# tijiang13/InstantAvatar

Hardware: NVIDIA H100
Metric: rays/sec at 512x512 render (higher is better)
Workload: dtype f32 geometry + f16 hash-grid/MLP (fp32 accumulate)

## Files before the change

### instantavatar_b200/csrc/ia_host.h

```cpp
#pragma once
#include <cuda_runtime.h>
#include <stdio.h>

#include "../../include/ia_b200.h"

char* ia_err_buf();

inline int ia_set_err(int code, const char* fmt, const char* detail = "") {
    snprintf(ia_err_buf(), 512, fmt, detail);
    return code;
}
#define set_err ia_set_err
#define IA_CHECK_CUDA(expr)                                                                        \
    do {                                                                                           \
        cudaError_t _e = (expr);                                                                   \
        if (_e != cudaSuccess) return ia_set_err(IA_ECUDA, #expr ": %s", cudaGetErrorString(_e)); \
    } while (0)
#define IA_REQUIRE(cond)                                                        \
    do {                                                                        \
        if (!(cond)) return ia_set_err(IA_EINVAL, "invalid argument: %s", #cond); \
    } while (0)

constexpr int kMaxDevices = 64;
inline int current_device() {
    int dev = 0;
    if (cudaGetDevice(&dev) != cudaSuccess) return -1;
    return dev;
}

inline int sm_count() {
    static int g_sm_count[kMaxDevices] = {};
    const int dev = current_device();
    if (dev < 0) return 0;
    int& c = g_sm_count[dev % kMaxDevices];
    if (!c) cudaDeviceGetAttribute(&c, cudaDevAttrMultiProcessorCount, dev);
    return c;
}

struct PerDeviceFlag {
    bool done[kMaxDevices] = {};
    bool get() const { const int d = current_device(); return d >= 0 && done[d % kMaxDevices]; }
    void set() { const int d = current_device(); if (d >= 0) done[d % kMaxDevices] = true; }
};

template <auto Kernel>
inline int allow_dynamic_smem(int bytes) {
    static PerDeviceFlag done;
    if (!done.get()) {
        IA_CHECK_CUDA(cudaFuncSetAttribute(Kernel, cudaFuncAttributeMaxDynamicSharedMemorySize, bytes));
        done.set();
    }
    return IA_OK;
}
```

### instantavatar_b200/csrc/ia_kernels.cu

```cuda
#include <math.h>
#include <stdio.h>
#include <string.h>

#include <type_traits>

#include "ia_warp_eval.cuh"

using namespace ia;

static int g_render_rays = 4;

constexpr int kRenderWarps = 12;

#include "ia_host.h"
#include "ia_scene.cuh"

static thread_local char g_err[512] = "";
char* ia_err_buf() { return g_err; }

struct RenderArgs {
    SceneDev sd;
    const float* rays_o; const float* rays_d; const float* near; const float* far; const float* bg;
    int n_rays, image_width;
    float* rgb; float* depth; float* alpha; float* counter;
    int* tile_counter;
    IaStats* stats;
    const int* tile_order;
    const int* n_active;
    const int* gidx; float* const* peer_rgba; int n_peers;
};

__device__ __forceinline__ void peer_store_rgba(const RenderArgs& a, int ray, float r, float g, float b, float al) {
    if (!a.peer_rgba) return;
    const long px = a.gidx ? a.gidx[ray] : ray;
    const float4 v = make_float4(r, g, b, al);
    for (int p = 0; p < a.n_peers; p++) reinterpret_cast<float4*>(a.peer_rgba[p])[px] = v;
}

struct RenderWarpExtra {
    float qx[64], qy[64], qz[64], qt[64];
    int qowner[64];
    float bt[32];
    int bo[32];
};

template <bool kNV = false>
struct RenderSmem {
    __align__(128) uint32_t occ[64 * 64 * 64 / 32];
    __align__(16) __half W[kMlpHalfs];
    FrameConst fc;
    __align__(8) uint64_t mbar;
    std::conditional_t<kNV, WarpScratchNV, WarpScratch<false>> ws[kRenderWarps];
    RenderWarpExtra wx[kRenderWarps];
};

__device__ __forceinline__ void occupied_interval(const FrameConst& fc, const int* __restrict__ cbox, int G, float ox,
                                                  float oy, float oz, float dx, float dy, float dz, float& t0, float& t1) {
    t0 = -INFINITY; t1 = INFINITY;
    const float o[3] = {ox, oy, oz}, d[3] = {dx, dy, dz};
#pragma unroll
    for (int a = 0; a < 3; a++) {
        const float cell = 1.0f / fc.occ_s[a];
        float lo = -INFINITY, hi = INFINITY;
        if (cbox[a] > 0) lo = fc.occ_min[a] + ((float)cbox[a] - 0.5f) * cell;
        if (cbox[3 + a] < G - 1) hi = fc.occ_min[a] + ((float)cbox[3 + a] + 1.5f) * cell;
        if (fabsf(d[a]) < 1e-12f) {
            if (o[a] < lo || o[a] > hi) { t0 = INFINITY; t1 = -INFINITY; }
        } else {
            const float inv = 1.0f / d[a];
            float ta = (lo - o[a]) * inv, tb = (hi - o[a]) * inv;
            if (ta > tb) { const float tmp = ta; ta = tb; tb = tmp; }
            if (ta == ta) t0 = fmaxf(t0, ta);
            if (tb == tb) t1 = fminf(t1, tb);
        }
    }
}

struct FrameRay {
    float ox = 0, oy = 0, oz = 0, dx = 0, dy = 0, dz = 1, t = 0, far = 0, dt = 0;
    int kbeg = 0, kend = -1;
};

__device__ __forceinline__ bool load_ray(const RenderArgs& a, const FrameConst& fc, const int* __restrict__ cbox, int G, int ray,
                                         FrameRay& r) {
    r.ox = a.rays_o[ray * 3]; r.oy = a.rays_o[ray * 3 + 1]; r.oz = a.rays_o[ray * 3 + 2];
    r.dx = a.rays_d[ray * 3]; r.dy = a.rays_d[ray * 3 + 1]; r.dz = a.rays_d[ray * 3 + 2];
    r.t = a.near[ray]; r.far = a.far[ray];
    r.dt = (r.far - r.t) / (float)IA_MAX_SAMPLES;
    float t0, t1;
    occupied_interval(fc, cbox, G, r.ox, r.oy, r.oz, r.dx, r.dy, r.dz, t0, t1);
    if (!(cbox[6] != 0 && t0 <= t1 && r.dt > 0.f)) return false;
    const float k0f = floorf((fmaxf(t0, r.t) - r.t) / r.dt) - 2.f, k1f = ceilf((fminf(t1, r.far) - r.t) / r.dt) + 2.f;
    r.kbeg = (int)fminf(fmaxf(k0f, 0.f), 1024.f);
    r.kend = (int)fminf(fmaxf(k1f, -1.f), 1024.f);
    return true;
}

__device__ __forceinline__ void store_ray(const RenderArgs& a, int ray, float Cr, float Cg, float Cb, float T, float Dp, float n) {
    float b0 = 1.f, b1 = 1.f, b2 = 1.f;
    if (a.bg) { b0 = a.bg[ray * 3]; b1 = a.bg[ray * 3 + 1]; b2 = a.bg[ray * 3 + 2]; }
    const float r = Cr + T * b0, g = Cg + T * b1, b = Cb + T * b2, al = 1.0f - T;
    a.rgb[ray * 3 + 0] = r; a.rgb[ray * 3 + 1] = g; a.rgb[ray * 3 + 2] = b;
    a.depth[ray] = Dp; a.alpha[ray] = al; a.counter[ray] = n;
    peer_store_rgba(a, ray, r, g, b, al);
}

__host__ __device__ constexpr int tile_width(int rays) { return rays >= 2 ? 2 : 1; }

template <int kRays>
__device__ __forceinline__ int tile_ray(int tile, int rl, bool tiled, int image_width) {
    constexpr int kTileW = tile_width(kRays);
    if (tiled) {
        const int tiles_x = image_width / kTileW;
        const int ty = tile / tiles_x, tx = tile % tiles_x;
        return (ty * (kRays / kTileW) + rl / kTileW) * image_width + tx * kTileW + (rl % kTileW);
    }
    return tile * kRays + rl;
}

template <int kRays, bool kNV = false>
__global__ void __launch_bounds__(256) render_plan_kernel(const __grid_constant__ RenderArgs a, int* __restrict__ cost) {
    __shared__ FrameConst fc;
    load_frame_const<kNV>(fc, a.sd);
    __syncthreads();
    constexpr int kTileW = tile_width(kRays);
    constexpr int kTileH = kRays / kTileW;
    const int G = a.sd.s.G;
    const uint32_t* occ = a.sd.s.occ_bits;
    const int* cbox = reinterpret_cast<const int*>(occ + G * G * G / 32);
    const bool tiled = a.image_width > 0 && (a.image_width % kTileW) == 0 && (a.n_rays % (a.image_width * kTileH)) == 0;
    const int n_tiles = (a.n_rays + kRays - 1) / kRays;
    const int gid = blockIdx.x * blockDim.x + threadIdx.x;
    const int tile = gid / kRays, rl = gid % kRays;
    int cnt = 0, ray = -1;
    if (tile < n_tiles) {
        ray = tile_ray<kRays>(tile, rl, tiled, a.image_width);
        if (ray < a.n_rays) {
            FrameRay r;
            if (load_ray(a, fc, cbox, G, ray, r)) {
                float t = r.t;
                for (int i = 0; i < r.kbeg; i++) t += r.dt;
                for (int k = r.kbeg; k <= r.kend && t < r.far; k++) {
                    const float x = __fmaf_rn(t, r.dx, r.ox), y = __fmaf_rn(t, r.dy, r.oy), z = __fmaf_rn(t, r.dz, r.oz);
                    cnt += occupied<true>(occ, fc.occ_min, fc.occ_s, G, x, y, z);
                    t += r.dt;
                }
            }
        } else {
            ray = -1;
        }
    }
    int tot = cnt;
#pragma unroll
    for (int o = 1; o < kRays; o <<= 1) tot += __shfl_xor_sync(kFull, tot, o);
    if (tile < n_tiles) {
        if (rl == 0) cost[tile] = tot;
        if (tot == 0 && ray >= 0) store_ray(a, ray, 0.f, 0.f, 0.f, 1.f, 0.f, 0.f);
    }
}

__global__ void __launch_bounds__(1024) order_tiles_kernel(const int* __restrict__ cost, int n_tiles, int* __restrict__ order,
                                                           int* __restrict__ n_active) {
    __shared__ int hist[256];
    __shared__ int offs[256];
    constexpr int kPer = 16;
    for (int i = threadIdx.x; i < 256; i += blockDim.x) hist[i] = 0;
    __syncthreads();
    auto bucket = [](int c) { return 255 - min(255, c >> 2); };
    for (int base = 0; base < n_tiles; base += 1024 * kPer) {
        int c[kPer];
#pragma unroll
        for (int j = 0; j < kPer; j++) { const int i = base + j * 1024 + threadIdx.x; c[j] = i < n_tiles ? cost[i] : 0; }
#pragma unroll
        for (int j = 0; j < kPer; j++) if (c[j] > 0) atomicAdd(&hist[bucket(c[j])], 1);
    }
    __syncthreads();
    if (threadIdx.x < 32) {
        int loc[8], sum = 0;
#pragma unroll
        for (int j = 0; j < 8; j++) { loc[j] = hist[threadIdx.x * 8 + j]; sum += loc[j]; }
        int incl = sum;
        for (int o = 1; o < 32; o <<= 1) { const int y = __shfl_up_sync(0xffffffffu, incl, o); if ((int)threadIdx.x >= o) incl += y; }
        int acc = incl - sum;
#pragma unroll
        for (int j = 0; j < 8; j++) { offs[threadIdx.x * 8 + j] = acc; acc += loc[j]; }
        if (threadIdx.x == 31) *n_active = incl;
    }
    __syncthreads();
    for (int base = 0; base < n_tiles; base += 1024 * kPer) {
        int c[kPer];
#pragma unroll
        for (int j = 0; j < kPer; j++) { const int i = base + j * 1024 + threadIdx.x; c[j] = i < n_tiles ? cost[i] : 0; }
#pragma unroll
        for (int j = 0; j < kPer; j++)
            if (c[j] > 0) order[atomicAdd(&offs[bucket(c[j])], 1)] = base + j * 1024 + threadIdx.x;
    }
}

template <int kRays, bool kNV = false>
__global__ void __launch_bounds__(kRenderWarps * 32, 1) render_fwd_kernel(const __grid_constant__ RenderArgs a) {
    constexpr int kDepth = 32 / kRays;
    constexpr int kTileW = tile_width(kRays);
    constexpr int kTileH = kRays / kTileW;
    extern __shared__ __align__(128) unsigned char smem_raw[];
    RenderSmem<kNV>& sm = *reinterpret_cast<RenderSmem<kNV>*>(smem_raw);
    const int lane = threadIdx.x & 31, warp = threadIdx.x >> 5;
    const int G = a.sd.s.G;
    const EvalCtx ctx = stage_frame<kNV>(a.sd, sm.fc, sm.W, &sm.mbar, sm.occ);
    auto& ws = sm.ws[warp];
    RenderWarpExtra& wx = sm.wx[warp];
    const FrameConst& fc = sm.fc;
    const int* cbox = reinterpret_cast<const int*>(a.sd.s.occ_bits + G * G * G / 32);

    const bool tiled = a.image_width > 0 && (a.image_width % kTileW) == 0 && (a.n_rays % (a.image_width * kTileH)) == 0;
    const int n_tiles = (a.n_rays + kRays - 1) / kRays;
    const int rl = lane % kRays, jl = lane / kRays;
    WorkCounters wc;

    for (;;) {
        int tile = 0;
        if (lane == 0) {
            tile = atomicAdd(a.tile_counter, 1);
            if (a.tile_order) tile = tile < *a.n_active ? a.tile_order[tile] : n_tiles;
        }
        tile = __shfl_sync(kFull, tile, 0);
        if (tile >= n_tiles) break;
        const int ray = tile_ray<kRays>(tile, rl, tiled, a.image_width);
        const bool has = ray < a.n_rays;
        FrameRay r;
        int k = jl;
        if (has) {
            if (load_ray(a, fc, cbox, G, ray, r)) k = (r.kbeg / kDepth) * kDepth + jl;
            for (int i = 0; i < k; i++) r.t += r.dt;
        }
        const float ox = r.ox, oy = r.oy, oz = r.oz, dx = r.dx, dy = r.dy, dz = r.dz, far = r.far, dt = r.dt;
        const int kend = r.kend;
        float t = r.t;
        float T = 1.f, Cr = 0.f, Cg = 0.f, Cb = 0.f, Dp = 0.f;
        int nocc = 0;
        int qhead = 0, qcount = 0;
        for (;;) {
            const bool dead = __shfl_sync(kFull, !(T > 1e-4f), rl);
            while (qcount < 32) {
                const bool act = has && !dead && k <= kend && t < far;
                if (!__any_sync(kFull, act)) break;
                bool occ = false;
                float x = 0, y = 0, z = 0;
                if (act) {
                    x = __fmaf_rn(t, dx, ox); y = __fmaf_rn(t, dy, oy); z = __fmaf_rn(t, dz, oz);
                    occ = occupied<false>(sm.occ, fc.occ_min, fc.occ_s, G, x, y, z);
                }
                const unsigned m = __ballot_sync(kFull, occ);
                if (occ) {
                    const int slot = (qhead + qcount + __popc(m & ((1u << lane) - 1u))) & 63;
                    wx.qx[slot] = x; wx.qy[slot] = y; wx.qz[slot] = z; wx.qt[slot] = t; wx.qowner[slot] = rl;
                    nocc++;
                }
                qcount += __popc(m);
                if (act) {
#pragma unroll
                    for (int i = 0; i < kDepth; i++) t += dt;
                    k += kDepth;
                }
            }
            if (qcount == 0) break;
            __syncwarp();
            const int n = min(qcount, 32);
            const int slot = (qhead + lane) & 63;
            float sx = 0, sy = 0, sz = 0, stt = 0;
            int sown = 0;
            if (lane < n) { sx = wx.qx[slot]; sy = wx.qy[slot]; sz = wx.qz[slot]; stt = wx.qt[slot]; sown = wx.qowner[slot]; }
            const bool owner_dead = __shfl_sync(kFull, !(T > 1e-4f), sown);
            const bool sact = lane < n && !owner_dead;
            qhead = (qhead + n) & 63;
            qcount -= n;
            if (!__any_sync(kFull, sact)) continue;
            wc.samples += sact ? 1u : 0u;
            SampleOut so;
            if constexpr (kNV) {
                warp_eval_nv(ctx, a.sd.nv, ws, sact, sx, sy, sz, true, lane, so, wc.net_evals, wc.hash_loads);
            } else {
                warp_eval_samples<false>(ctx, ws, sact, sx, sy, sz, true, lane, so, wc.gathers, wc.net_evals, wc.field_loads,
                                         wc.hash_loads);
            }
            ws.res[lane][0] = so.sigma; ws.res[lane][1] = so.r; ws.res[lane][2] = so.g; ws.res[lane][3] = so.b;
            wx.bt[lane] = stt; wx.bo[lane] = sact ? sown : -1;
            __syncwarp();
            for (int i = 0; i < n; i++) {
                if (wx.bo[i] == lane && T > 1e-4f) {
                    const float tau = expf(-ws.res[i][0] * dt);
                    const float al = 1.0f - tau;
                    if (!(al < 0.01f)) {
                        const float w = al * T;
                        Cr = __fmaf_rn(w, ws.res[i][1], Cr);
                        Cg = __fmaf_rn(w, ws.res[i][2], Cg);
                        Cb = __fmaf_rn(w, ws.res[i][3], Cb);
                        Dp = __fmaf_rn(w, wx.bt[i], Dp);
                        T *= tau;
                    }
                }
            }
            __syncwarp();
        }
#pragma unroll
        for (int o = kRays; o < 32; o <<= 1) nocc += __shfl_xor_sync(kFull, nocc, o);
        if (has && jl == 0) {
            store_ray(a, ray, Cr, Cg, Cb, T, Dp, (float)nocc);
            wc.rays_hit += nocc > 0 ? 1u : 0u;
        }
    }
    wc.flush(a.stats, lane);
}

struct QueryArgs {
    SceneDev sd;
    const float* pts; int n; int eval_mode;
    float* rgb; float* sigma; float* xc_best; int8_t* best_init;
    IaStats* stats;
    int* batch_counter;
    const int* n_dev; const int* index;
};

template <int kWarps, bool kKeepXc, bool kNV = false>
struct QuerySmem {
    __align__(16) __half W[kMlpHalfs];
    FrameConst fc;
    __align__(8) uint64_t mbar;
    std::conditional_t<kNV, WarpScratchNV, WarpScratch<kKeepXc>> ws[kWarps];
};

template <int kWarps, bool kKeepXc, bool kNV = false>
__global__ void __launch_bounds__(kWarps * 32, 1) deform_query_kernel(const __grid_constant__ QueryArgs a) {
    extern __shared__ __align__(128) unsigned char smem_raw[];
    QuerySmem<kWarps, kKeepXc, kNV>& sm = *reinterpret_cast<QuerySmem<kWarps, kKeepXc, kNV>*>(smem_raw);
    const int lane = threadIdx.x & 31, warp = threadIdx.x >> 5;
    const EvalCtx ctx = stage_frame<kNV>(a.sd, sm.fc, sm.W, &sm.mbar);
    WorkCounters wc;
    const int n_pts = a.n_dev ? min(*a.n_dev, a.n) : a.n;
    int k = 1;
    if (kKeepXc && !kNV && a.n_dev) {
        const int n_warps = gridDim.x * kWarps, n32 = (n_pts + 31) / 32;
        k = 4 * n32 * 4 <= 5 * n_warps ? 4 : (4 * n32 * 2 <= 5 * n_warps ? 2 : 1);
    }
    const int spw = 32 / k;
    const int n_batches = (n_pts + spw - 1) / spw;
    for (int bidx = blockIdx.x * kWarps + warp;; bidx += gridDim.x * kWarps) {
        if (a.batch_counter) {
            int nb = 0;
            if (lane == 0) nb = atomicAdd(a.batch_counter, 1);
            bidx = __shfl_sync(kFull, nb, 0);
        }
        if (bidx >= n_batches) break;
        const int p = bidx * spw + (lane & (spw - 1));
        bool act = p < n_pts;
        const bool owner = lane < spw;
        long q = p;
        if (act && a.index) q = a.index[p];
        float x = 0, y = 0, z = 0;
        if (act) { x = a.pts[q * 3]; y = a.pts[q * 3 + 1]; z = a.pts[q * 3 + 2]; }
        SampleOut so;
        if constexpr (kNV) {
            warp_eval_nv(ctx, a.sd.nv, sm.ws[warp], act, x, y, z, a.eval_mode != 0, lane, so, wc.net_evals, wc.hash_loads);
        } else if constexpr (kKeepXc) {
            warp_eval_samples<kKeepXc>(ctx, sm.ws[warp], act, x, y, z, a.eval_mode != 0, lane, so, wc.gathers, wc.net_evals,
                                       wc.field_loads, wc.hash_loads, k);
        } else {
            warp_eval_samples<kKeepXc>(ctx, sm.ws[warp], act, x, y, z, a.eval_mode != 0, lane, so, wc.gathers, wc.net_evals,
                                       wc.field_loads, wc.hash_loads);
        }
        act = act && owner;
        wc.samples += act ? 1u : 0u;
        if (act) {
            a.sigma[q] = so.sigma;
            a.rgb[q * 3] = so.r; a.rgb[q * 3 + 1] = so.g; a.rgb[q * 3 + 2] = so.b;
            if constexpr (kKeepXc) {
                if (a.xc_best) { a.xc_best[q * 3] = so.xc[0]; a.xc_best[q * 3 + 1] = so.xc[1]; a.xc_best[q * 3 + 2] = so.xc[2]; }
            }
            if (a.best_init) a.best_init[q] = (int8_t)so.best;
        }
    }
    wc.flush(a.stats, lane);
}

struct OccRoot { float x, y, z; int cell; };

struct OccArgs {
    SceneDev sd;
    const float* grid_jitter; const float* grid_aabb; int G, passes;
    int* counters;
    float* cand;
    OccRoot* roots;
    int batch_first, batch_stride;
    float* density_max;
    float* const* peer_density; int n_peers;
    IaStats* stats;
};

constexpr int kOccRootWarps = 8;
constexpr int kOccRootCtas = 2;
constexpr int kOccRootMaxCtas = 320;
constexpr int kOccNetWarps = 8;
constexpr int kOccNetCtas = 4;

constexpr size_t kOccCandBytes = 256 + sizeof(float) * 3 * kNumInit * 32 * kOccRootWarps * kOccRootMaxCtas;

__host__ __device__ inline int occ_cells_per_batch(int passes) { return 32 / passes; }
__host__ __device__ inline int occ_batches(int G, int passes) {
    return (G * G * G + occ_cells_per_batch(passes) - 1) / occ_cells_per_batch(passes);
}

template <bool kNV>
__global__ void __launch_bounds__(kOccRootWarps * 32, kOccRootCtas) occupancy_roots_kernel(const __grid_constant__ OccArgs a) {
    static_assert(kOccRootWarps * 32 >= kNumInit * 12, "load_frame_const stages the bone transforms one thread per entry");
    __shared__ FrameConst fc;
    load_frame_const<kNV>(fc, a.sd);
    __syncthreads();
    const int lane = threadIdx.x & 31, warp = threadIdx.x >> 5;
    FieldDesc field;
    field.data = a.sd.s.field; field.D = a.sd.s.D; field.H = a.sd.s.H; field.W = a.sd.s.W;
    WorkCounters wc;
    float (*cand)[kNumInit][32] =
        reinterpret_cast<float (*)[kNumInit][32]>(a.cand + (size_t)(blockIdx.x * kOccRootWarps + warp) * 3 * kNumInit * 32);
    const int G = a.G, n3g = G * G * G;
    const int cells_per_batch = occ_cells_per_batch(a.passes);
    const int n_batches = occ_batches(G, a.passes);
    for (;;) {
        int lidx = 0;
        if (lane == 0) lidx = atomicAdd(&a.counters[0], 1);
        lidx = __shfl_sync(kFull, lidx, 0);
        const int bidx = a.batch_first + lidx * a.batch_stride;
        if (bidx >= n_batches) break;
        const int cell = bidx * cells_per_batch + lane / a.passes;
        const int pass = lane % a.passes;
        const bool act = lane < cells_per_batch * a.passes && cell < n3g;
        float x = 0, y = 0, z = 0;
        if (act) {
            const int ci = cell / (G * G), cj = (cell / G) % G, ck = cell % G;
            const float* jit = a.grid_jitter + ((long)pass * n3g + cell) * 3;
            const float fG = (float)G;
            x = ((float)ci / fG + jit[0] / fG) * (a.grid_aabb[3] - a.grid_aabb[0]) + a.grid_aabb[0];
            y = ((float)cj / fG + jit[1] / fG) * (a.grid_aabb[4] - a.grid_aabb[1]) + a.grid_aabb[1];
            z = ((float)ck / fG + jit[2] / fG) * (a.grid_aabb[5] - a.grid_aabb[2]) + a.grid_aabb[2];
        }
        wc.samples += act ? 1u : 0u;
        unsigned kept = 0;
        float xc[3] = {0.f, 0.f, 0.f};
        if constexpr (kNV) {
            if (act) {
                float d2;
                const int v = nv_nearest(a.sd.nv, x, y, z, d2);
                if (v >= 0) { nv_apply(a.sd.nv, v, x, y, z, xc); kept = 1u; }
            }
        } else {
            kept = warp_find_roots<false>(field, fc, cand, act, x, y, z, lane, wc.gathers, wc.field_loads);
        }
        int total;
        int pos = warp_excl_scan(__popc(kept), lane, total);
        int base = 0;
        if (lane == 0 && total) base = atomicAdd(&a.counters[1], total);
        pos += __shfl_sync(kFull, base, 0);
        wc.net_evals += __popc(kept);
        for (unsigned m = kept; m; m &= m - 1) {
            const int b = __ffs(m) - 1;
            OccRoot r;
            if constexpr (kNV) { r.x = xc[0]; r.y = xc[1]; r.z = xc[2]; }
            else { r.x = cand[0][b][lane]; r.y = cand[1][b][lane]; r.z = cand[2][b][lane]; }
            r.cell = cell;
            a.roots[pos++] = r;
        }
        __syncwarp();
    }
    wc.flush(a.stats, lane);
}

template <bool kNanToNum>
__global__ void __launch_bounds__(kOccNetWarps * 32, kOccNetCtas) occupancy_net_kernel(const __grid_constant__ OccArgs a) {
    __shared__ __align__(16) __half W[kW3Off];
    __shared__ __align__(16) __half At[kOccNetWarps][32][kW1Stride];
    __shared__ float cs[6];
    const int lane = threadIdx.x & 31, warp = threadIdx.x >> 5;
    for (int i = threadIdx.x; i < kW3Off / 2; i += blockDim.x)
        reinterpret_cast<uint32_t*>(W)[i] = reinterpret_cast<const uint32_t*>(a.sd.s.mlp_h)[i];
    if (threadIdx.x < 3) { cs[threadIdx.x] = a.sd.s.net_center[threadIdx.x]; cs[3 + threadIdx.x] = a.sd.s.net_scale[threadIdx.x]; }
    __syncthreads();
    const __half2* table = reinterpret_cast<const __half2*>(a.sd.s.table_h);
    const int n = a.counters[1];
    const int g = lane >> 2, t = lane & 3;
    WorkCounters wc;
    for (int base = (blockIdx.x * kOccNetWarps + warp) * 32; base < n; base += gridDim.x * kOccNetWarps * 32) {
        const int r = base + lane;
        int cell = -1;
        float nrm[3];
        feature_row(reinterpret_cast<__half2*>(&At[warp][lane][0]), table, a.sd.hl, cs, cs + 3, r < n, [&](float x[3]) {
            const float4 v = reinterpret_cast<const float4*>(a.roots)[r];
            cell = __float_as_int(v.w);
            x[0] = v.x; x[1] = v.y; x[2] = v.z;
        }, nrm, &wc.hash_loads);
        __syncwarp();
#pragma unroll
        for (int mt = 0; mt < 2; mt++) {
            float o[2][4];
            mlp_density_tile16(&At[warp][16 * mt][0], W, lane, o);
            const int cA = __shfl_sync(kFull, cell, 16 * mt + g), cB = __shfl_sync(kFull, cell, 16 * mt + g + 8);
            if (t == 0) {
                float s[2] = {__low2float(__floats2half2_rn(o[0][0], o[0][1])), __low2float(__floats2half2_rn(o[0][2], o[0][3]))};
                const int c[2] = {cA, cB};
#pragma unroll
                for (int h = 0; h < 2; h++) {
                    if (kNanToNum && !isfinite(s[h])) s[h] = 0.f;
                    if (c[h] >= 0 && s[h] > 0.f) {
                        if (a.peer_density) {
                            for (int pr = 0; pr < a.n_peers; pr++) atomicMax(reinterpret_cast<int*>(a.peer_density[pr]) + c[h], __float_as_int(s[h]));
                        } else {
                            atomicMax(reinterpret_cast<int*>(a.density_max) + c[h], __float_as_int(s[h]));
                        }
                    }
                }
            }
        }
        __syncwarp();
    }
    wc.flush(a.stats, lane);
}

__global__ void __launch_bounds__(256) broyden_kernel(SceneDev sd, const float* __restrict__ xd, int n,
                                                      float* __restrict__ xc, uint8_t* __restrict__ valid,
                                                      float* __restrict__ jinv) {
    __shared__ FrameConst fc;
    load_frame_const(fc, sd);
    __syncthreads();
    FieldDesc f;
    f.data = sd.s.field; f.D = sd.s.D; f.H = sd.s.H; f.W = sd.s.W;
    const int p = blockIdx.x * blockDim.x + threadIdx.x;
    if (p >= n) return;
    const float t0 = xd[p * 3], t1 = xd[p * 3 + 1], t2 = xd[p * 3 + 2];
    float xs[kNumInit][3];
    unsigned vmask = 0;
#pragma unroll 1
    for (int b = 0; b < kNumInit; b++) {
        float J[9];
        int ng = 0;
        const bool ok = broyden_solve(f, fc.bp, fc.Tb[b], t0, t1, t2, xs[b], jinv ? J : nullptr, ng);
        if (ok) vmask |= 1u << b;
        if (jinv) {
            for (int k = 0; k < 9; k++) jinv[((long)p * kNumInit + b) * 9 + k] = ok ? J[k] : 0.f;
        }
    }
    unsigned kept = vmask;
    for (int i = 0; i < kNumInit - 1; i++) {
        if (!((vmask >> i) & 1)) continue;
        for (int j = i + 1; j < kNumInit; j++) {
            if (!((vmask >> j) & 1)) continue;
            const float d0 = xs[i][0] - xs[j][0], d1 = xs[i][1] - xs[j][1], d2 = xs[i][2] - xs[j][2];
            if (dot3f(d0, d0, d1, d1, d2, d2) < fc.filter_thr) { kept &= ~(1u << i); break; }
        }
// ... 258 lines not shown
    }
    return set_err(IA_EINVAL, "unknown option: %s", name);
}

int ia_hashgrid_layout(uint32_t res[IA_NUM_LEVELS], float scale[IA_NUM_LEVELS], uint32_t size[IA_NUM_LEVELS],
                       uint32_t offset[IA_NUM_LEVELS], uint32_t* total_entries) {
    HashLevels hl;
    uint32_t tot;
    host_hash_levels(hl, &tot);
    for (int l = 0; l < kLevels; l++) {
        if (res) res[l] = hl.res[l];
        if (scale) scale[l] = hl.scale[l];
        if (size) size[l] = hl.size[l];
        if (offset) offset[l] = hl.offset[l];
    }
    if (total_entries) *total_entries = tot;
    return IA_OK;
}

int ia_precompute(const float* voxel_w, const float* tfs, const float* offset_k, const float* scale_k, int D, int H,
                  int W, float* field_out, float* voxel_d_out, float* aabb_out, ia_stream_t stream) {
    IA_REQUIRE(voxel_w && tfs && offset_k && scale_k && field_out);
    IA_REQUIRE(D > 1 && H > 1 && W > 1);
    IA_REQUIRE((long)D * H * (W + 1) <= 0xffffffffL);
    const long V = (long)D * H * W;
    if (aabb_out) aabb_init_kernel<<<1, 32, 0, (cudaStream_t)stream>>>(aabb_out);
    precompute_kernel<<<(unsigned)((V + 255) / 256), 256, 0, (cudaStream_t)stream>>>(
        voxel_w, tfs, offset_k, scale_k, D, H, W, field_out, voxel_d_out, aabb_out);
    IA_CHECK_CUDA(cudaPeekAtLastError());
    return IA_OK;
}

int ia_params_to_half(const float* enc_params, const float* col_params, void* table_h, void* mlp_h, ia_stream_t stream) {
    IA_REQUIRE(enc_params && col_params && table_h && mlp_h);
    HashLevels hl;
    uint32_t tot;
    host_hash_levels(hl, &tot);
    params_to_half_kernel<float><<<(tot + 255) / 256, 256, 0, (cudaStream_t)stream>>>(
        enc_params, col_params, reinterpret_cast<__half2*>(table_h), reinterpret_cast<__half*>(mlp_h), tot);
    IA_CHECK_CUDA(cudaPeekAtLastError());
    return IA_OK;
}

int ia_mlp_to_half(const float* enc_params, const float* col_params, void* mlp_h, ia_stream_t stream) {
    IA_REQUIRE(enc_params && col_params && mlp_h);
    params_to_half_kernel<float><<<(kMlpAllHalfs + 255) / 256, 256, 0, (cudaStream_t)stream>>>(enc_params, col_params, nullptr,
                                                                                             reinterpret_cast<__half*>(mlp_h), 0);
    IA_CHECK_CUDA(cudaPeekAtLastError());
    return IA_OK;
}

int ia_mlp_to_half_from_half(const void* enc_mlp_h, const void* col_h, void* mlp_h, ia_stream_t stream) {
    IA_REQUIRE(enc_mlp_h && col_h && mlp_h);
    params_to_half_kernel<__half><<<(kMlpAllHalfs + 255) / 256, 256, 0, (cudaStream_t)stream>>>(
        reinterpret_cast<const __half*>(enc_mlp_h), reinterpret_cast<const __half*>(col_h), nullptr, reinterpret_cast<__half*>(mlp_h), 0);
    IA_CHECK_CUDA(cudaPeekAtLastError());
    return IA_OK;
}

int ia_pack_occupancy(const uint8_t* field_bool, uint32_t* bits, int G, ia_stream_t stream) {
    IA_REQUIRE(field_bool && bits && G >= 32 && G % 32 == 0);
    const int n_words = G * G * G / 32;
    pack_init_box_kernel<<<1, 32, 0, (cudaStream_t)stream>>>(bits, n_words, G);
    pack_occupancy_kernel<<<(n_words + 255) / 256, 256, 0, (cudaStream_t)stream>>>(field_bool, bits, n_words, G);
    IA_CHECK_CUDA(cudaPeekAtLastError());
    return IA_OK;
}

size_t ia_render_workspace_bytes(int n_rays) { return 256 + 2 * sizeof(int) * (size_t)(n_rays + 1); }

}

template <int kRays, bool kNV = false>
static int launch_render(RenderArgs& a, bool plan, int* ws_cost, int* ws_order, cudaStream_t st) {
    const size_t smem = sizeof(RenderSmem<kNV>);
    if (const int rc = allow_dynamic_smem<render_fwd_kernel<kRays, kNV>>((int)smem)) return rc;
    const int n_tiles = (a.n_rays + kRays - 1) / kRays;
    int grid = sm_count();
    if (grid <= 0) return set_err(IA_ECUDA, "no CUDA device%s");
    grid = min(grid, (n_tiles + kRenderWarps - 1) / kRenderWarps);
    if (plan) {
        const long threads = (long)n_tiles * kRays;
        render_plan_kernel<kRays, kNV><<<(unsigned)((threads + 255) / 256), 256, 0, st>>>(a, ws_cost);
        order_tiles_kernel<<<1, 1024, 0, st>>>(ws_cost, n_tiles, ws_order, a.tile_counter + 1);
        a.tile_order = ws_order;
        a.n_active = a.tile_counter + 1;
    }
    render_fwd_kernel<kRays, kNV><<<grid, kRenderWarps * 32, smem, st>>>(a);
    return IA_OK;
}

template <int kWarps, bool kKeepXc, bool kNV = false>
static int launch_query_t(QueryArgs& a, cudaStream_t stream) {
    const size_t smem = sizeof(QuerySmem<kWarps, kKeepXc, kNV>);
    if (const int rc = allow_dynamic_smem<deform_query_kernel<kWarps, kKeepXc, kNV>>((int)smem)) return rc;
    const int n_batches = (a.n + 31) / 32;
    int grid = sm_count();
    if (grid <= 0) return set_err(IA_ECUDA, "no CUDA device%s");
    grid = min(grid, (n_batches + kWarps - 1) / kWarps);
    deform_query_kernel<kWarps, kKeepXc, kNV><<<grid, kWarps * 32, smem, stream>>>(a);
    IA_CHECK_CUDA(cudaPeekAtLastError());
    return IA_OK;
}

static int launch_query(QueryArgs& a, cudaStream_t stream) {
    if (a.sd.s.nv) {
        if (a.xc_best) return launch_query_t<12, true, true>(a, stream);
        return launch_query_t<12, false, true>(a, stream);
    }
    if (a.xc_best) return launch_query_t<12, true>(a, stream);
    return launch_query_t<12, false>(a, stream);
}

extern "C" {

static int render_fwd_impl(const IaScene* scene, const float* rays_o, const float* rays_d, const float* near, const float* far,
                           int n_rays, const float* bg, int image_width, float* rgb, float* depth, float* alpha, float* counter,
                           void* workspace, size_t workspace_bytes, IaStats* stats, const int* peer_gidx, float* const* peer_rgba,
                           int n_peers, ia_stream_t stream) {
    IA_REQUIRE(n_rays >= 0);
    if (n_rays == 0) return IA_OK;
    IA_REQUIRE(rays_o && rays_d && near && far && rgb && depth && alpha && counter && workspace);
    RenderArgs a;
    int rc = make_scene_dev(scene, a.sd, true);
    if (rc) return rc;
    a.rays_o = rays_o; a.rays_d = rays_d; a.near = near; a.far = far; a.bg = bg;
    a.n_rays = n_rays; a.image_width = image_width;
    a.rgb = rgb; a.depth = depth; a.alpha = alpha; a.counter = counter;
    IA_REQUIRE(workspace_bytes >= 256);
    a.tile_counter = reinterpret_cast<int*>(workspace);
    a.stats = stats;
    a.tile_order = nullptr; a.n_active = nullptr;
    a.gidx = peer_gidx; a.peer_rgba = peer_rgba; a.n_peers = n_peers;
    cudaStream_t st = (cudaStream_t)stream;
    IA_CHECK_CUDA(cudaMemsetAsync(workspace, 0, 256, st));
    const bool plan = workspace_bytes >= ia_render_workspace_bytes(n_rays);
    int* ws_cost = reinterpret_cast<int*>(reinterpret_cast<char*>(workspace) + 256);
    int* ws_order = ws_cost + (n_rays + 1);
    if (scene->nv) {
        rc = launch_render<4, true>(a, plan, ws_cost, ws_order, st);
        if (rc) return rc;
        IA_CHECK_CUDA(cudaPeekAtLastError());
        return IA_OK;
    }
    switch (g_render_rays) {
        case 2: rc = launch_render<2>(a, plan, ws_cost, ws_order, st); break;
        case 1: rc = launch_render<1>(a, plan, ws_cost, ws_order, st); break;
        default: rc = launch_render<4>(a, plan, ws_cost, ws_order, st); break;
    }
    if (rc) return rc;
    IA_CHECK_CUDA(cudaPeekAtLastError());
    return IA_OK;
}

int ia_render_fwd(const IaScene* scene, const float* rays_o, const float* rays_d, const float* near, const float* far,
                  int n_rays, const float* bg, int image_width, float* rgb, float* depth, float* alpha, float* counter,
                  void* workspace, size_t workspace_bytes, IaStats* stats, ia_stream_t stream) {
    return render_fwd_impl(scene, rays_o, rays_d, near, far, n_rays, bg, image_width, rgb, depth, alpha, counter, workspace,
                           workspace_bytes, stats, nullptr, nullptr, 0, stream);
}

int ia_render_fwd_peer(const IaScene* scene, const float* rays_o, const float* rays_d, const float* near, const float* far,
                       int n_rays, const float* bg, int image_width, float* rgb, float* depth, float* alpha, float* counter,
                       void* workspace, size_t workspace_bytes, IaStats* stats, const int* pixel_index,
                       float* const* peer_rgba, int n_peers, ia_stream_t stream) {
    IA_REJECT_NV(scene, "ia_render_fwd_peer");
    IA_REQUIRE(peer_rgba && n_peers >= 1 && n_peers <= 64);
    return render_fwd_impl(scene, rays_o, rays_d, near, far, n_rays, bg, image_width, rgb, depth, alpha, counter, workspace,
                           workspace_bytes, stats, pixel_index, peer_rgba, n_peers, stream);
}

int ia_deform_query(const IaScene* scene, const float* pts, int n, int eval_mode, float* rgb, float* sigma,
                    float* xc_best, int8_t* best_init, IaStats* stats, ia_stream_t stream) {
    IA_REQUIRE(n >= 0);
    if (n == 0) return IA_OK;
    IA_REQUIRE(pts && rgb && sigma);
    QueryArgs a;
    int rc = make_scene_dev(scene, a.sd, false);
    if (rc) return rc;
    a.pts = pts; a.n = n; a.eval_mode = eval_mode; a.rgb = rgb; a.sigma = sigma; a.xc_best = xc_best;
    a.best_init = best_init; a.stats = stats;
    a.batch_counter = nullptr;
    a.n_dev = nullptr; a.index = nullptr;
    return launch_query(a, (cudaStream_t)stream);
}

__attribute__((visibility("hidden"))) int ia_internal_query_list(const IaScene* scene, const float* pts, const int* index,
                                                                 const int* n_dev, int capacity, int eval_mode, float* rgb,
                                                                 float* sigma, float* xc_best, int8_t* best_init,
                                                                 int* batch_counter, IaStats* stats, ia_stream_t stream) {
    IA_REQUIRE(pts && index && n_dev && capacity > 0 && rgb && sigma && xc_best && batch_counter);
    QueryArgs a;
    int rc = make_scene_dev(scene, a.sd, false);
    if (rc) return rc;
    a.pts = pts; a.n = capacity; a.eval_mode = eval_mode; a.rgb = rgb; a.sigma = sigma; a.xc_best = xc_best;
    a.best_init = best_init; a.stats = stats;
    a.batch_counter = batch_counter;
    a.n_dev = n_dev; a.index = index;
    return launch_query(a, (cudaStream_t)stream);
}

static int occupancy_query_impl(const IaScene* scene, const float* jitter, const float* aabb, int G, int passes,
                                float* density_max, float* const* peer_density, int n_peers, void* workspace, int shard,
                                int n_shards, IaStats* stats, ia_stream_t stream) {
    IA_REQUIRE(jitter && aabb && (density_max || peer_density) && workspace && G > 0 && G <= 1024 && passes > 0 && passes <= 32);
    IA_REQUIRE(n_shards >= 1 && shard >= 0 && shard < n_shards);
    OccArgs a;
    int rc = make_scene_dev(scene, a.sd, false);
    if (rc) return rc;
    a.grid_jitter = jitter; a.grid_aabb = aabb; a.G = G; a.passes = passes;
    a.counters = reinterpret_cast<int*>(workspace);
    a.cand = reinterpret_cast<float*>(reinterpret_cast<char*>(workspace) + 256);
    a.roots = reinterpret_cast<OccRoot*>(reinterpret_cast<char*>(workspace) + kOccCandBytes);
    a.batch_first = shard; a.batch_stride = n_shards;
    a.density_max = density_max; a.peer_density = peer_density; a.n_peers = n_peers;
    a.stats = stats;
    cudaStream_t st = (cudaStream_t)stream;
    const int sms = sm_count();
    if (sms <= 0) return set_err(IA_ECUDA, "no CUDA device%s");
    IA_CHECK_CUDA(cudaMemsetAsync(workspace, 0, 256, st));
    if (!peer_density) IA_CHECK_CUDA(cudaMemsetAsync(density_max, 0, sizeof(float) * G * G * G, st));
    const int n_batches = (occ_batches(G, passes) - shard + n_shards - 1) / n_shards;
    const int roots_grid = min(min(sms * kOccRootCtas, kOccRootMaxCtas), (n_batches + kOccRootWarps - 1) / kOccRootWarps);
    if (roots_grid > 0) {
        if (scene->nv) occupancy_roots_kernel<true><<<roots_grid, kOccRootWarps * 32, 0, st>>>(a);
        else occupancy_roots_kernel<false><<<roots_grid, kOccRootWarps * 32, 0, st>>>(a);
        IA_CHECK_CUDA(cudaPeekAtLastError());
    }
    if (scene->nv) occupancy_net_kernel<false><<<sms * kOccNetCtas, kOccNetWarps * 32, 0, st>>>(a);
    else occupancy_net_kernel<true><<<sms * kOccNetCtas, kOccNetWarps * 32, 0, st>>>(a);
    IA_CHECK_CUDA(cudaPeekAtLastError());
    return IA_OK;
}

extern "C" size_t ia_occupancy_query_workspace_bytes(int G, int passes, int n_shards) {
    if (G <= 0 || G > 1024 || passes <= 0 || passes > 32 || n_shards < 1) return 0;
    const long batches = (occ_batches(G, passes) + n_shards - 1) / n_shards;
    return kOccCandBytes + sizeof(OccRoot) * (size_t)batches * (size_t)(occ_cells_per_batch(passes) * passes) * kNumInit;
}

extern "C" int ia_occupancy_query(const IaScene* scene, const float* jitter, const float* aabb, int G, int passes,
                                  float* density_max, void* workspace, int shard, int n_shards, IaStats* stats,
                                  ia_stream_t stream) {
    return occupancy_query_impl(scene, jitter, aabb, G, passes, density_max, nullptr, 0, workspace, shard, n_shards, stats, stream);
}

extern "C" int ia_occupancy_query_peer(const IaScene* scene, const float* jitter, const float* aabb, int G, int passes,
                                       float* const* peer_density, int n_peers, void* workspace, int shard, int n_shards,
                                       IaStats* stats, ia_stream_t stream) {
    IA_REJECT_NV(scene, "ia_occupancy_query_peer");
    IA_REQUIRE(peer_density && n_peers >= 1 && n_peers <= 64);
    return occupancy_query_impl(scene, jitter, aabb, G, passes, nullptr, peer_density, n_peers, workspace, shard, n_shards, stats, stream);
}

int ia_broyden(const IaScene* scene, const float* xd, int n, float* xc, uint8_t* valid, float* j_inv, ia_stream_t stream) {
    IA_REJECT_NV(scene, "ia_broyden");
    IA_REQUIRE(n >= 0);
    if (n == 0) return IA_OK;
    IA_REQUIRE(xd && xc && valid);
    SceneDev sd;
    int rc = make_scene_dev(scene, sd, false, false);
    if (rc) return rc;
    broyden_kernel<<<(n + 255) / 256, 256, 0, (cudaStream_t)stream>>>(sd, xd, n, xc, valid, j_inv);
    IA_CHECK_CUDA(cudaPeekAtLastError());
    return IA_OK;
}

int ia_tcnn_encoder_forward(const IaScene* scene, const float* x01, int n, void* out16_h, ia_stream_t stream) {
    IA_REQUIRE(n >= 0);
    if (n == 0) return IA_OK;
    IA_REQUIRE(x01 && out16_h && scene && scene->table_h && scene->mlp_h);
    SceneDev sd;
    sd.s = *scene;
    host_hash_levels(sd.hl, nullptr);
    sd.filter_thr = 0.f;
    constexpr int kW = 8;
    const int n_batches = (n + 31) / 32;
    const int grid = min(sm_count() * 4, (n_batches + kW - 1) / kW);
    if (grid <= 0) return set_err(IA_ECUDA, "no CUDA device%s");
    tcnn_encoder_forward_kernel<kW><<<grid, kW * 32, 0, (cudaStream_t)stream>>>(sd, x01, n, reinterpret_cast<__half*>(out16_h));
    IA_CHECK_CUDA(cudaPeekAtLastError());
    return IA_OK;
}

int ia_tcnn_mlp_forward(const void* mlp_h, const float* in15, int n, void* out3_h, ia_stream_t stream) {
    IA_REQUIRE(n >= 0);
    if (n == 0) return IA_OK;
    IA_REQUIRE(mlp_h && in15 && out3_h);
    constexpr int kW = 8;
    const int n_tiles = (n + 15) / 16;
    const int grid = min(sm_count() * 4, (n_tiles + kW - 1) / kW);
    if (grid <= 0) return set_err(IA_ECUDA, "no CUDA device%s");
    tcnn_mlp_forward_kernel<kW><<<grid, kW * 32, 0, (cudaStream_t)stream>>>(reinterpret_cast<const __half*>(mlp_h), in15, n,
                                                                            reinterpret_cast<__half*>(out3_h));
    IA_CHECK_CUDA(cudaPeekAtLastError());
    return IA_OK;
}

int ia_ngp_forward(const IaScene* scene, const float* x, int n, float* sigma, float* rgb, ia_stream_t stream) {
    IA_REQUIRE(n >= 0);
    if (n == 0) return IA_OK;
    IA_REQUIRE(x && sigma && rgb);
    IA_REQUIRE(scene && scene->table_h && scene->mlp_h && scene->net_center && scene->net_scale);
    SceneDev sd;
// ... 14 lines not shown
```

### instantavatar_b200/csrc/ia_occupancy.cu

```cuda
#include <math.h>
#include <stdint.h>

#include "ia_host.h"
#include "ia_union_find.cuh"

namespace {

constexpr int kThreads = 256;

struct OccWork {
    float* pooled;
    int* parent;
    int* count;
    double* sum;
    unsigned long long* best;
};

__global__ void pool_kernel(const float* __restrict__ density, int G, float* __restrict__ pooled, double* __restrict__ sum) {
    const int i = blockIdx.x * blockDim.x + threadIdx.x;
    const int N = G * G * G;
    float v = 0.f;
    if (i < N) {
        const int x = i / (G * G), y = (i / G) % G, z = i % G;
        float m = -INFINITY;
// ... 12 lines not shown
    for (int o = 16; o; o >>= 1) s += __shfl_xor_sync(0xffffffffu, s, o);
    __shared__ double red[kThreads / 32];
    if ((threadIdx.x & 31) == 0) red[threadIdx.x >> 5] = s;
    __syncthreads();
    if (threadIdx.x == 0) {
        double t = 0;
        for (int w = 0; w < kThreads / 32; w++) t += red[w];
        atomicAdd(sum, t);
    }
}

__global__ void threshold_kernel(const float* __restrict__ pooled, int N, int G, const double* __restrict__ sum,
                                 int* __restrict__ parent, int* __restrict__ count) {
    const int i = blockIdx.x * blockDim.x + threadIdx.x;
    if (i >= N) return;
    const float mean = (float)(*sum / (double)N);
    const float thr = fminf(mean, 0.01f);
    const bool on = pooled[i] > thr;
    const bool next_on = on && ((i % G) < G - 1) && pooled[i + 1] > thr;
    parent[i] = on ? (next_on ? i + 1 : i) : -1;
    count[i] = 0;
}

__global__ void union_kernel(int* __restrict__ parent, int G) {
    const int i = blockIdx.x * blockDim.x + threadIdx.x;
    const int N = G * G * G;
    if (i >= N || parent[i] < 0) return;
    const int x = i / (G * G), y = (i / G) % G, z = i % G;
    for (int dx = 0; dx <= 1; dx++)
        for (int dy = -1; dy <= 1; dy++)
            for (int dz = -1; dz <= 1; dz++) {
                if (dx == 0 && (dy < 0 || (dy == 0 && dz <= 1))) continue;
                const int xx = x + dx, yy = y + dy, zz = z + dz;
                if (xx >= G || yy < 0 || yy >= G || zz < 0 || zz >= G) continue;
                const int j = (xx * G + yy) * G + zz;
                if (parent[j] >= 0) uf_union(parent, i, j);
            }
}

__global__ void flatten_count_kernel(int* __restrict__ parent, int* __restrict__ count, int N) {
    const int i = blockIdx.x * blockDim.x + threadIdx.x;
    if (i >= N || parent[i] < 0) return;
    const int r = uf_root(parent, i);
    parent[i] = r;
    atomicAdd(&count[r], 1);
}

__global__ void argmax_kernel(const int* __restrict__ count, int N, unsigned long long* __restrict__ best) {
    const int i = blockIdx.x * blockDim.x + threadIdx.x;
    unsigned long long key = 0;
    if (i < N && count[i] > 0) key = ((unsigned long long)count[i] << 32) | (unsigned long long)(0xffffffffu - (unsigned)i);
    for (int o = 16; o; o >>= 1) {
        const unsigned long long other = __shfl_xor_sync(0xffffffffu, key, o);
        key = other > key ? other : key;
    }
    if ((threadIdx.x & 31) == 0 && key) atomicMax(best, key);
}

__global__ void select_pack_kernel(const int* __restrict__ parent, int G, const unsigned long long* __restrict__ best,
                                   uint8_t* __restrict__ field, uint32_t* __restrict__ bits) {
    const int i = blockIdx.x * blockDim.x + threadIdx.x;
    const int N = G * G * G;
    const unsigned long long b = *best;
    const int label = b ? (int)(0xffffffffu - (unsigned)(b & 0xffffffffu)) : -2;
    bool on = false;
    if (i < N) {
        on = parent[i] == label;
        if (field) field[i] = on ? 1 : 0;
    }
    const unsigned m = __ballot_sync(0xffffffffu, on);
    if ((threadIdx.x & 31) == 0 && i < N) {
        bits[i >> 5] = m;
        if (m) {
            int* box = reinterpret_cast<int*>(bits + N / 32);
            const int x = i / (G * G), y = (i / G) % G, z0 = i % G;
            atomicMin(&box[0], x); atomicMax(&box[3], x);
            atomicMin(&box[1], y); atomicMax(&box[4], y);
            atomicMin(&box[2], z0 + (__ffs(m) - 1)); atomicMax(&box[5], z0 + (31 - __clz(m)));
            box[6] = 1;
        }
    }
}

__global__ void init_box_kernel(uint32_t* bits, int n_words, int G) {
    int* box = reinterpret_cast<int*>(bits + n_words);
    if (threadIdx.x < 8) box[threadIdx.x] = threadIdx.x < 3 ? G : (threadIdx.x < 6 ? -1 : 0);
}

}

extern "C" int ia_occupancy_build(const float* density, int G, uint8_t* field_out, uint32_t* bits_out, void* workspace,
                                  size_t workspace_bytes, ia_stream_t stream) {
    IA_REQUIRE(density && bits_out && workspace);
    IA_REQUIRE(G >= 32 && G % 32 == 0);
    const int N = G * G * G;
    const size_t need = (size_t)N * 12 + 64;
    IA_REQUIRE(workspace_bytes >= need);
    cudaStream_t st = (cudaStream_t)stream;
    char* ws = reinterpret_cast<char*>(workspace);
    float* pooled = reinterpret_cast<float*>(ws);
    int* parent = reinterpret_cast<int*>(ws + (size_t)N * 4);
    int* count = reinterpret_cast<int*>(ws + (size_t)N * 8);
    double* sum = reinterpret_cast<double*>(ws + (size_t)N * 12);
    unsigned long long* best = reinterpret_cast<unsigned long long*>(ws + (size_t)N * 12 + 8);
    IA_CHECK_CUDA(cudaMemsetAsync(sum, 0, 16, st));
    init_box_kernel<<<1, 32, 0, st>>>(bits_out, N / 32, G);
    const int blocks = (N + kThreads - 1) / kThreads;
    pool_kernel<<<blocks, kThreads, 0, st>>>(density, G, pooled, sum);
    threshold_kernel<<<blocks, kThreads, 0, st>>>(pooled, N, G, sum, parent, count);
    union_kernel<<<blocks, kThreads, 0, st>>>(parent, G);
    flatten_count_kernel<<<blocks, kThreads, 0, st>>>(parent, count, N);
    argmax_kernel<<<blocks, kThreads, 0, st>>>(count, N, best);
    select_pack_kernel<<<blocks, kThreads, 0, st>>>(parent, G, best, field_out, bits_out);
    IA_CHECK_CUDA(cudaPeekAtLastError());
    return IA_OK;
}
```

Baseline: 84.81 million.

## Overlap render kernel prologue with tile ordering via programmatic dependent launch

```diff
diff --git a/instantavatar_b200/csrc/ia_host.h b/instantavatar_b200/csrc/ia_host.h
--- a/instantavatar_b200/csrc/ia_host.h
+++ b/instantavatar_b200/csrc/ia_host.h
@@ -52,3 +52,20 @@
     }
     return IA_OK;
 }
+
+template <typename... KArgs, typename... Args>
+inline cudaError_t launch_dependent(void (*kernel)(KArgs...), unsigned grid, unsigned block, size_t smem, cudaStream_t st,
+                                    Args... args) {
+    cudaLaunchAttribute attr[1];
+    attr[0].id = cudaLaunchAttributeProgrammaticStreamSerialization;
+    attr[0].val.programmaticStreamSerializationAllowed = 1;
+    cudaLaunchConfig_t cfg = {};
+    cfg.gridDim = dim3(grid); cfg.blockDim = dim3(block); cfg.dynamicSmemBytes = smem; cfg.stream = st;
+    cfg.attrs = attr; cfg.numAttrs = 1;
+    return cudaLaunchKernelEx(&cfg, kernel, args...);
+}
+
+#ifdef __CUDACC__
+__device__ __forceinline__ void pdl_wait() { asm volatile("griddepcontrol.wait;" ::: "memory"); }
+__device__ __forceinline__ void pdl_launch_dependents() { asm volatile("griddepcontrol.launch_dependents;" ::: "memory"); }
+#endif
diff --git a/instantavatar_b200/csrc/ia_kernels.cu b/instantavatar_b200/csrc/ia_kernels.cu
--- a/instantavatar_b200/csrc/ia_kernels.cu
+++ b/instantavatar_b200/csrc/ia_kernels.cu
@@ -17,6 +17,36 @@
 
 static thread_local char g_err[512] = "";
 char* ia_err_buf() { return g_err; }
+
+#ifdef IA_CTA_TIMES
+constexpr int kCtaTimesMax = 1024;
+__device__ unsigned long long g_cta_times[2][kCtaTimesMax][2];
+__device__ int g_cta_grid[2];
+__device__ __forceinline__ unsigned long long globaltimer_ns() {
+    unsigned long long t;
+    asm volatile("mov.u64 %0, %%globaltimer;" : "=l"(t));
+    return t;
+}
+#define IA_CTA_ENTRY(slot)                                                                              \
+    do {                                                                                                \
+        if (threadIdx.x == 0 && blockIdx.x < kCtaTimesMax) g_cta_times[slot][blockIdx.x][0] = globaltimer_ns(); \
+        if (threadIdx.x == 0 && blockIdx.x == 0) g_cta_grid[slot] = gridDim.x;                          \
+    } while (0)
+#define IA_CTA_EXIT(slot)                                                                               \
+    do {                                                                                                \
+        __syncthreads();                                                                                \
+        if (threadIdx.x == 0 && blockIdx.x < kCtaTimesMax) g_cta_times[slot][blockIdx.x][1] = globaltimer_ns(); \
+    } while (0)
+extern "C" int ia_debug_cta_times(int slot, unsigned long long* out, int* grid) {
+    IA_REQUIRE(slot == 0 || slot == 1);
+    IA_CHECK_CUDA(cudaMemcpyFromSymbol(out, g_cta_times, sizeof(g_cta_times[0]), sizeof(g_cta_times[0]) * slot));
+    IA_CHECK_CUDA(cudaMemcpyFromSymbol(grid, g_cta_grid, sizeof(int), sizeof(int) * slot));
+    return IA_OK;
+}
+#else
+#define IA_CTA_ENTRY(slot) do {} while (0)
+#define IA_CTA_EXIT(slot) do {} while (0)
+#endif
 
 struct RenderArgs {
     SceneDev sd;
@@ -160,7 +190,8 @@
 }
 
 __global__ void __launch_bounds__(1024) order_tiles_kernel(const int* __restrict__ cost, int n_tiles, int* __restrict__ order,
-                                                           int* __restrict__ n_active) {
+                                                           int* __restrict__ counter) {
+    pdl_launch_dependents();
     __shared__ int hist[256];
     __shared__ int offs[256];
     constexpr int kPer = 16;
@@ -184,7 +215,7 @@
         int acc = incl - sum;
 #pragma unroll
         for (int j = 0; j < 8; j++) { offs[threadIdx.x * 8 + j] = acc; acc += loc[j]; }
-        if (threadIdx.x == 31) *n_active = incl;
+        if (threadIdx.x == 31) { counter[0] = 0; counter[1] = incl; }
     }
     __syncthreads();
     for (int base = 0; base < n_tiles; base += 1024 * kPer) {
@@ -206,7 +237,9 @@
     RenderSmem<kNV>& sm = *reinterpret_cast<RenderSmem<kNV>*>(smem_raw);
     const int lane = threadIdx.x & 31, warp = threadIdx.x >> 5;
     const int G = a.sd.s.G;
+    IA_CTA_ENTRY(1);
     const EvalCtx ctx = stage_frame<kNV>(a.sd, sm.fc, sm.W, &sm.mbar, sm.occ);
+    pdl_wait();
     auto& ws = sm.ws[warp];
     RenderWarpExtra& wx = sm.wx[warp];
     const FrameConst& fc = sm.fc;
@@ -310,6 +343,7 @@
         }
     }
     wc.flush(a.stats, lane);
+    IA_CTA_EXIT(1);
 }
 
 struct QueryArgs {
@@ -409,9 +443,16 @@
     return (G * G * G + occ_cells_per_batch(passes) - 1) / occ_cells_per_batch(passes);
 }
 
+__global__ void occ_clear_kernel(int* __restrict__ counters, float* __restrict__ density, int n) {
+    const int i = blockIdx.x * blockDim.x + threadIdx.x;
+    if (i < 64) counters[i] = 0;
+    if (density && i < n) density[i] = 0.f;
+}
+
 template <bool kNV>
 __global__ void __launch_bounds__(kOccRootWarps * 32, kOccRootCtas) occupancy_roots_kernel(const __grid_constant__ OccArgs a) {
     static_assert(kOccRootWarps * 32 >= kNumInit * 12, "load_frame_const stages the bone transforms one thread per entry");
+    IA_CTA_ENTRY(0);
     __shared__ FrameConst fc;
     load_frame_const<kNV>(fc, a.sd);
     __syncthreads();
@@ -471,6 +512,7 @@
         __syncwarp();
     }
     wc.flush(a.stats, lane);
+    IA_CTA_EXIT(0);
 }
 
 template <bool kNanToNum>
@@ -895,11 +937,13 @@
     if (plan) {
         const long threads = (long)n_tiles * kRays;
         render_plan_kernel<kRays, kNV><<<(unsigned)((threads + 255) / 256), 256, 0, st>>>(a, ws_cost);
-        order_tiles_kernel<<<1, 1024, 0, st>>>(ws_cost, n_tiles, ws_order, a.tile_counter + 1);
+        order_tiles_kernel<<<1, 1024, 0, st>>>(ws_cost, n_tiles, ws_order, a.tile_counter);
         a.tile_order = ws_order;
         a.n_active = a.tile_counter + 1;
-    }
-    render_fwd_kernel<kRays, kNV><<<grid, kRenderWarps * 32, smem, st>>>(a);
+    } else {
+        IA_CHECK_CUDA(cudaMemsetAsync(a.tile_counter, 0, 256, st));
+    }
+    IA_CHECK_CUDA(launch_dependent(render_fwd_kernel<kRays, kNV>, grid, kRenderWarps * 32, smem, st, a));
     return IA_OK;
 }
 
@@ -946,7 +990,6 @@
     a.tile_order = nullptr; a.n_active = nullptr;
     a.gidx = peer_gidx; a.peer_rgba = peer_rgba; a.n_peers = n_peers;
     cudaStream_t st = (cudaStream_t)stream;
-    IA_CHECK_CUDA(cudaMemsetAsync(workspace, 0, 256, st));
     const bool plan = workspace_bytes >= ia_render_workspace_bytes(n_rays);
     int* ws_cost = reinterpret_cast<int*>(reinterpret_cast<char*>(workspace) + 256);
     int* ws_order = ws_cost + (n_rays + 1);
@@ -1031,8 +1074,8 @@
     cudaStream_t st = (cudaStream_t)stream;
     const int sms = sm_count();
     if (sms <= 0) return set_err(IA_ECUDA, "no CUDA device%s");
-    IA_CHECK_CUDA(cudaMemsetAsync(workspace, 0, 256, st));
-    if (!peer_density) IA_CHECK_CUDA(cudaMemsetAsync(density_max, 0, sizeof(float) * G * G * G, st));
+    const int n_cells = peer_density ? 0 : G * G * G;
+    occ_clear_kernel<<<max(1, (n_cells + 255) / 256), 256, 0, st>>>(a.counters, peer_density ? nullptr : density_max, n_cells);
     const int n_batches = (occ_batches(G, passes) - shard + n_shards - 1) / n_shards;
     const int roots_grid = min(min(sms * kOccRootCtas, kOccRootMaxCtas), (n_batches + kOccRootWarps - 1) / kOccRootWarps);
     if (roots_grid > 0) {
diff --git a/instantavatar_b200/csrc/ia_occupancy.cu b/instantavatar_b200/csrc/ia_occupancy.cu
--- a/instantavatar_b200/csrc/ia_occupancy.cu
+++ b/instantavatar_b200/csrc/ia_occupancy.cu
@@ -118,9 +118,10 @@
     }
 }
 
-__global__ void init_box_kernel(uint32_t* bits, int n_words, int G) {
+__global__ void init_box_kernel(uint32_t* bits, int n_words, int G, double* sum, unsigned long long* best) {
     int* box = reinterpret_cast<int*>(bits + n_words);
     if (threadIdx.x < 8) box[threadIdx.x] = threadIdx.x < 3 ? G : (threadIdx.x < 6 ? -1 : 0);
+    if (threadIdx.x == 0) { *sum = 0.0; *best = 0ull; }
 }
 
 }
@@ -139,8 +140,7 @@
     int* count = reinterpret_cast<int*>(ws + (size_t)N * 8);
     double* sum = reinterpret_cast<double*>(ws + (size_t)N * 12);
     unsigned long long* best = reinterpret_cast<unsigned long long*>(ws + (size_t)N * 12 + 8);
-    IA_CHECK_CUDA(cudaMemsetAsync(sum, 0, 16, st));
-    init_box_kernel<<<1, 32, 0, st>>>(bits_out, N / 32, G);
+    init_box_kernel<<<1, 32, 0, st>>>(bits_out, N / 32, G, sum, best);
     const int blocks = (N + kThreads - 1) / kThreads;
     pool_kernel<<<blocks, kThreads, 0, st>>>(density, G, pooled, sum);
     threshold_kernel<<<blocks, kThreads, 0, st>>>(pooled, N, G, sum, parent, count);
```

Result: no change. 85.08 million (median of 6 runs) (+0.3%).
